# VikParuchuri/surya

Measured on AMD Instinct MI355X. Metric: text-lines/sec recognised (whole node), higher is better.
Workload: dtype bf16; 1 GPU; RecognitionPredictor device loop, 256 ragged 64x{128..512} crops/GPU, batch 256, max_tokens=48, REC-FULL synthetic weights (conditioned recipe, seed 0), tiles resident in HBM; parallelism=1 GPU, weights=conditioned

## Files before the change

### include/surya_amd.h

```cpp
#ifndef SURYA_AMD_H
#define SURYA_AMD_H
#include <stddef.h>
#include <stdint.h>

#ifdef __cplusplus
extern "C" {
#endif

#define SA_OK 0
#define SA_ERR_ARG (-1)
#define SA_ERR_SHAPE (-2)
#define SA_ERR_UNSUPPORTED (-3)
#define SA_ERR_STATE (-4)
#define SA_ERR_NOMEM (-5)

#define SA_DTYPE_F32 0
#define SA_DTYPE_BF16 1

const char* surya_amd_version(void);

typedef struct surya_rec_config {
    int32_t enc_depth, enc_hidden, enc_inter, enc_inter_pad, enc_heads;
    int32_t patch_dim, patch_dim_pad;
    int32_t merge;
    int32_t window_tokens;
    int32_t enc_out_hidden;
    uint32_t fullatt_mask;
    float enc_eps;
    int32_t vocab, dec_hidden, dec_inter, dec_layers, dec_heads, dec_kv_heads, dec_head_dim;
    float dec_eps;
    int32_t bbox_size, embed_multiplier;
    int32_t image_token_id, pad_token_id, eos_token_id;
    int32_t max_slots;
    int32_t max_kv_len;
    int32_t max_patches;
    int32_t max_prefill_tokens;
    int32_t dtype;
} surya_rec_config;

enum {
    SA_RW_PATCH = 0, SA_RW_MERGER_LN, SA_RW_FC1_W, SA_RW_FC1_B, SA_RW_FC2_W, SA_RW_FC2_B, SA_RW_IMG_H, SA_RW_IMG_W,
    SA_RW_DEC_NORM, SA_RW_TOK_EMBED, SA_RW_LM_W, SA_RW_LM_B, SA_RW_BBOX_W, SA_RW_BBOX_B, SA_RW_ENC_INVFREQ,
    SA_RW_DEC_INVFREQ, SA_RW_GLOBALS
};
enum { SA_RE_NORM1 = 0, SA_RE_QKV_W, SA_RE_QKV_B, SA_RE_PROJ_W, SA_RE_PROJ_B, SA_RE_NORM2, SA_RE_GU_W, SA_RE_GU_B,
       SA_RE_DOWN_W, SA_RE_DOWN_B, SA_RE_COUNT };
enum { SA_RD_LN1 = 0, SA_RD_QKV_W, SA_RD_QKV_B, SA_RD_O_W, SA_RD_LN2, SA_RD_GU_W, SA_RD_DOWN_W, SA_RD_COUNT };
#define SA_RW_ENC(l, k) (SA_RW_GLOBALS + (l) * SA_RE_COUNT + (k))
#define SA_RW_DEC(cfg_enc_depth, l, k) (SA_RW_GLOBALS + (cfg_enc_depth) * SA_RE_COUNT + (l) * SA_RD_COUNT + (k))
#define SA_RW_TOTAL(enc_depth, dec_layers) (SA_RW_GLOBALS + (enc_depth) * SA_RE_COUNT + (dec_layers) * SA_RD_COUNT)

typedef struct surya_rec surya_rec;

size_t surya_rec_workspace_bytes(const surya_rec_config* cfg);

int surya_rec_create(const surya_rec_config* cfg, const void* const* weights, int n_weights, surya_rec** out);
int surya_rec_destroy(surya_rec* h);

int surya_rec_plan_encoder(const surya_rec_config* cfg, const int32_t* grid_hw, int n_images, int32_t* src_row,
                           int32_t* pos_hw, int32_t* cu_window, int32_t* n_windows, int32_t* merged_src);

int surya_rec_prefill(surya_rec* h, const float* tiles, const int32_t* grid_hw, int n_images, const int32_t* input_ids,
                      const int32_t* seq_offsets, const int32_t* slot_ids, int n_seqs, void* stream);

int surya_rec_encode_ahead(surya_rec* h, const float* tiles, const int32_t* grid_hw, int n_images, void* stream);

int surya_rec_set_active(surya_rec* h, const int32_t* slots, int n_active, void* stream);

#define SA_MAX_STEPS 16
int surya_rec_decode(surya_rec* h, int n_steps, void* stream);

int surya_rec_read_outputs(surya_rec* h, int n_steps, int32_t* tokens, float* scores, int32_t* bboxes, void* stream);

int surya_rec_decode_async(surya_rec* h, int n_steps, int ring, void* stream);
int surya_rec_wait_outputs(surya_rec* h, int n_steps, int ring, int32_t* tokens, float* scores, int32_t* bboxes);

int surya_rec_preprocess(const uint8_t* pages, const void* lines, int n_lines, uint8_t* mask_arena, float* mid_arena, float* tiles,
                         int patch_size, int merge_size, float pad_value, const float* mean, const float* std, int any_poly,
                         int max_stage1_width, int pixel_stride, void* stream);

int surya_rec_encode_only(surya_rec* h, const float* tiles, const int32_t* grid_hw, int n_images, void* out, void* stream);
int surya_rec_copy_last_logits(surya_rec* h, float* dst, int max_rows, int* rows, void* stream);
int surya_rec_set_next_tokens(surya_rec* h, const int32_t* slots, const int32_t* tokens, int n, void* stream);

enum { SA_MX_QKV_W = 0, SA_MX_QKV_S, SA_MX_O_W, SA_MX_O_S, SA_MX_GU_W, SA_MX_GU_S, SA_MX_DOWN_W, SA_MX_DOWN_S, SA_MX_COUNT };
enum { SA_MX_LM_W = 0, SA_MX_LM_S, SA_MX_GLOBALS };
#define SA_MX_TOTAL(dec_layers) ((dec_layers) * SA_MX_COUNT + SA_MX_GLOBALS)
int surya_rec_set_mx_weights(surya_rec* h, const void* const* table, int n);

int surya_rec_set_kv_fp8(surya_rec* h, int on);

int surya_op_gemm(int dtype, int out_f32, int epi, const void* X, long ldx, const void* W, long ldw, void* C, long ldc,
                  const void* bias, const void* R, long ldr, int M, int N, int K, void* stream);
int surya_op_rmsnorm(int dtype, const void* x, long ldx, const void* w, void* y, long ldy, int rows, int C, float eps,
                     void* stream);
int surya_op_attn(int dtype, int head_dim, const void* q, const void* k, const void* v, void* out, const int32_t* seg_len,
                  const int64_t* q_off, const int64_t* k_off, const int64_t* v_off, const int64_t* o_off, int n_seg, int heads, int group,
                  int causal, float scale, long q_row, long q_head, long k_row, long k_head, long o_row, long o_head, void* stream);
int surya_op_decode_attn(int dtype, int head_dim, const float* qkv_part, int n_slabs, const void* qkv_bias, void* out, void* kcache,
                         void* vcache, const int32_t* active_slots, const int32_t* row_len, const float* rope_cs, int rows, int heads,
                         int kv_heads, int max_kv_len, float scale, void* stream);
int surya_op_kv8_quant_rows(int head_dim, const void* kcache, const void* vcache, const int32_t* tok_slot, const int32_t* tok_pos, int n_tokens,
                            void* k8, void* v8t, float* kscale, float* vscale, int kv_heads, int max_kv_len, void* stream);
int surya_op_decode_attn_kv8(int head_dim, const float* qkv_part, int n_slabs, const void* qkv_bias, void* out, void* k8, void* v8t,
                             float* kscale, float* vscale, const int32_t* active_slots, const int32_t* row_len, const float* rope_cs, int rows,
                             int heads, int kv_heads, int max_kv_len, float scale, void* stream);

int surya_op_mx_quantize(const float* x, int rows, int K, uint8_t* q, uint8_t* scales, void* stream);
int surya_op_gemm_mx(int mode, const uint8_t* X, const uint8_t* SX, const uint8_t* W, const uint8_t* SW, int M, int N, int K,
                     float* C, int* splitk, uint8_t* q_out, uint8_t* sq_out, void* stream);

enum { SA_DET_INPUT = 0,
       SA_DET_CONV,
       SA_DET_DWCONV,
       SA_DET_GROUPED1X1,
       SA_DET_LITEMLA,
       SA_DET_UPCAT,
       SA_DET_CLASSIFY,
       SA_DET_UPSAMPLE_OUT,
       SA_DET_UPSUM_SRC,
       SA_DET_UPSUM_CLASSIFY };
enum { SA_ACT_NONE = 0, SA_ACT_HSWISH = 1, SA_ACT_RELU = 2 };

typedef struct surya_det_op {
    int32_t type;
    int32_t in0, in1, out, res;
    int32_t cin, cout, k, stride, act;
    int32_t hin, win, hout, wout;
    int32_t w_idx, b_idx;
    int32_t p0, p1;
} surya_det_op;

typedef struct surya_det_config {
    int32_t n_ops, max_batch, height, width, num_labels, dtype;
} surya_det_config;

typedef struct surya_det surya_det;

int surya_det_create(const surya_det_config* cfg, const surya_det_op* ops, const void* const* weights, int n_weights,
                     const size_t* buf_elems, int n_bufs, surya_det** out);
int surya_det_destroy(surya_det* h);
int surya_det_forward(surya_det* h, const float* pixel_values, int batch, float* heatmaps, float* lowres, void* stream);
int surya_det_op_count(surya_det* h);
int surya_det_forward_timed(surya_det* h, const float* pixel_values, int batch, float* heatmaps, float* lowres, void* stream, float* op_ms,
                            int n_op_ms);
int surya_det_forward_u8(surya_det* h, const uint8_t* pixels_nhwc, int pixel_stride, const float* mean, const float* std, int batch,
                         float* heatmaps, float* lowres, void* stream);

int surya_resample_lanczos_u8(const uint8_t* src, int src_w, int src_h, int src_pix, uint8_t* dst, int dst_w, int dst_h, int dst_pix,
                              const int32_t* bounds_x, const int32_t* taps_x, int ksize_x, const int32_t* bounds_y,
                              const int32_t* taps_y, int ksize_y, uint8_t* tmp, void* stream);

size_t surya_det_boxes_workspace_bytes(int batch, int height, int width, int max_boxes);
int surya_det_boxes(const float* heat, long page_stride, int batch, int height, int width, float text_threshold, float low_text,
                    int max_boxes, float* boxes, float* conf, int32_t* count, void* workspace, size_t workspace_bytes, void* stream);

typedef struct surya_layout_config {
    int32_t img_h, img_w, patch, embed_dim, n_stages;
    int32_t depths[8], heads[8], kv_heads[8];
    int32_t window;
    float enc_eps;
    int32_t encoder_length;
    int32_t dec_layers, dec_hidden, dec_inter, dec_heads, dec_kv_heads;
    int32_t vocab, label_count, bbox_size;
    float rms_eps, ln_eps;
    int32_t max_batch, max_boxes, dtype;
    int32_t family, box_embed, category_count, merge_count;
} surya_layout_config;
enum { SA_FAMILY_LAYOUT = 0, SA_FAMILY_TABLE = 1 };

enum { SA_LW_PATCH_W = 0, SA_LW_PATCH_B, SA_LW_EMB_LN_W, SA_LW_EMB_LN_B, SA_LW_POS_EMB, SA_LW_DEC_FNORM, SA_LW_DEC_LN_W, SA_LW_DEC_LN_B,
       SA_LW_DEC_LM_W, SA_LW_DEC_BB_W, SA_LW_DEC_BB_B, SA_LW_DEC_INVFREQ, SA_LW_DEC_ZERO_BIAS, SA_LW_EMB_TABLES, SA_LW_GLOBALS = SA_LW_EMB_TABLES + 17 };
enum { SA_LS_SINCOS = 0, SA_LS_MERGE_NORM_W, SA_LS_MERGE_NORM_B, SA_LS_MERGE_RED_W, SA_LS_COUNT };
enum { SA_LB_LN1_W = 0, SA_LB_LN1_B, SA_LB_QKV_W, SA_LB_QKV_B, SA_LB_RELBIAS, SA_LB_PROJ_W, SA_LB_PROJ_B, SA_LB_LN2_W, SA_LB_LN2_B, SA_LB_FC1_W,
       SA_LB_FC1_B, SA_LB_FC2_W, SA_LB_FC2_B, SA_LB_COUNT };
enum { SA_LD_CNORM = 0, SA_LD_CQ_W, SA_LD_CKV_W, SA_LD_CO_W, SA_LD_CO_B, SA_LD_TNORM, SA_LD_QKV_W, SA_LD_TO_W, SA_LD_TO_B, SA_LD_MNORM, SA_LD_GU_W,
       SA_LD_DOWN_W, SA_LD_COUNT };

typedef struct surya_layout surya_layout;
int surya_layout_create(const surya_layout_config* cfg, const void* const* weights, int n_weights, surya_layout** out);
int surya_layout_destroy(surya_layout* h);
int surya_layout_encode(surya_layout* h, const float* pixel_values, int batch, void* stream);
int surya_layout_decode_step(surya_layout* h, const int32_t* boxes, int batch, int position, float* class_logits, float* bbox, void* stream);
int surya_layout_prefill(surya_layout* h, const int32_t* boxes, int batch, int n_tokens, float* class_logits, float* bbox, void* stream);
typedef struct surya_layout_feedback {
    int32_t skew_scaler;
    int32_t relabel_ids[2];
    int32_t head_widths[4];
    const int32_t* page_sizes;
} surya_layout_feedback;
int surya_layout_set_feedback(surya_layout* h, const surya_layout_feedback* fb, int batch, void* stream);
int surya_layout_decode_steps(surya_layout* h, const int32_t* boxes, int batch, int position, int n_steps, int ring, void* stream);
int surya_layout_wait_steps(surya_layout* h, int ring, int batch, int n_steps, float* class_logits, float* bbox, int32_t* fed_tokens);
int surya_layout_select(surya_layout* h, const int32_t* src_index, int n);
int surya_layout_encoder_states(surya_layout* h, void* out, int batch, void* stream);

int surya_prof_enable(int on);
int surya_set_tuning(const char* key, int value);
int surya_prof_read(int max_cfg, int* launches, double* ms, double* flops, double* bytes);
int surya_prof_read2(int max_cfg, int* launches, double* ms, double* flops, double* bytes, double* slab_bytes);
int surya_prof_event_overhead(void* stream, double* ms);

#ifdef __cplusplus
}
#endif
#endif
```

### surya_amd/csrc/common.h

```cpp
#pragma once
#include <hip/hip_runtime.h>
#include <cstdlib>
#include <stdint.h>
#include <stdio.h>

#include "../../include/surya_amd.h"

namespace sa {

typedef unsigned short bf16_t;
typedef __attribute__((ext_vector_type(4))) float f32x4;
typedef __attribute__((ext_vector_type(16))) float f32x16;
typedef __attribute__((ext_vector_type(8))) __bf16 bf16x8;
typedef unsigned int u32x4 __attribute__((ext_vector_type(4)));


#define SA_HIP(expr)                                                                                   \
    do {                                                                                               \
        hipError_t _e = (expr);                                                                        \
        if (_e != hipSuccess) {                                                                        \
            fprintf(stderr, "[surya_amd] %s:%d %s -> %s\n", __FILE__, __LINE__, #expr, hipGetErrorString(_e)); \
            return (int)_e;                                                                            \
        }                                                                                              \
    } while (0)
// ... 62 lines not shown
    v += dpp_mov<0x141>(v);
    v += dpp_mov<0x140>(v);
    return v;
}

__device__ __forceinline__ int mx_block_exp(float absmax) {
    if (!(absmax > 0.f)) return -127;
    int ex;
    const float f = frexpf(absmax, &ex);
    const int e = (f <= 0.875f) ? ex - 9 : ex - 8;
    return max(-127, min(127, e));
}
__device__ __forceinline__ uint32_t mx_pack4(float a, float b, float c, float d) {
    int r = __builtin_amdgcn_cvt_pk_fp8_f32(a, b, 0, false);
    r = __builtin_amdgcn_cvt_pk_fp8_f32(c, d, r, true);
    return (uint32_t)r;
}
template <int CTRL>
__device__ __forceinline__ float dpp_max(float v) { return fmaxf(v, dpp_mov<CTRL>(v)); }
__device__ __forceinline__ float quad_max(float v) { return dpp_max<0x4E>(dpp_max<0xB1>(v)); }
__device__ __forceinline__ float oct_max(float v) { return dpp_max<0x141>(quad_max(v)); }
__device__ __forceinline__ uint32_t mx_quant4_oct(const float (&v)[4], int& e8) {
    const float m = oct_max(fmaxf(fmaxf(fabsf(v[0]), fabsf(v[1])), fmaxf(fabsf(v[2]), fabsf(v[3]))));
    const int e = mx_block_exp(m);
    e8 = e + 127;
    return mx_pack4(ldexpf(v[0], -e), ldexpf(v[1], -e), ldexpf(v[2], -e), ldexpf(v[3], -e));
}

__device__ __forceinline__ float wave_sum(float v) {
#pragma unroll
    for (int o = 32; o > 0; o >>= 1) v += __shfl_xor(v, o, 64);
    return v;
}
__device__ __forceinline__ float wave_max(float v) {
#pragma unroll
    for (int o = 32; o > 0; o >>= 1) v = fmaxf(v, __shfl_xor(v, o, 64));
    return v;
}

__device__ __forceinline__ float silu_f(float x) { return x / (1.0f + __expf(-x)); }
template <typename TI>
__device__ __forceinline__ float silu_epi(float x) {
    if constexpr (sizeof(TI) == 2) return x * __builtin_amdgcn_rcpf(1.0f + __expf(-x));
    else return silu_f(x);
}
__device__ __forceinline__ float gelu_erf_f(float x) { return 0.5f * x * (1.0f + erff(x * 0.70710678118654752440f)); }
template <typename TI>
__device__ __forceinline__ float gelu_epi(float x) {
    if constexpr (sizeof(TI) == 2) {
        const float z = fabsf(x) * 0.70710678118654752440f;
        const float t = __builtin_amdgcn_rcpf(fmaf(0.3275911f, z, 1.0f));
        const float poly = t * fmaf(t, fmaf(t, fmaf(t, fmaf(t, 1.061405429f, -1.453152027f), 1.421413741f), -0.284496736f), 0.254829592f);
        const float erfc_abs = poly * __expf(-z * z);
        return 0.5f * x * (x < 0.f ? erfc_abs : 2.0f - erfc_abs);
    } else {
        return gelu_erf_f(x);
    }
}
__device__ __forceinline__ float gelu_tanh_f(float x) { return 0.5f * x * (1.0f + tanhf(0.7978845608028654f * (x + 0.044715f * x * x * x))); }
__device__ __forceinline__ float sigmoid_f(float x) { return 1.0f / (1.0f + __expf(-x)); }
__device__ __forceinline__ float hardswish_f(float x) {
    float t;
    asm("v_fma_f32 %0, %1, %2, 0.5 clamp" : "=v"(t) : "v"(x), "s"(1.0f / 6.0f));
    return x * t;
}
typedef float f32x2_hs __attribute__((ext_vector_type(2)));
__device__ __forceinline__ f32x2_hs hardswish_pk(f32x2_hs x) {
    f32x2_hs t;
    const f32x2_hs c = {1.0f / 6.0f, 1.0f / 6.0f};
    asm("v_pk_fma_f32 %0, %1, %2, 0.5 op_sel_hi:[1,0,0] clamp" : "=v"(t) : "v"(x), "s"(c));
    return x * t;
}

struct Tuning {
    int graph = 0;
    int split_target = 256;
    int split_min_kt = 4;
    int split_max = 8;
    int bigtile = 3;
    int bigtile_any = 0;
    int big_m_split = -1;
    int big_m_gateup = -1;
    int gateup_ring = 2;
    int conv_persist = 3;
    int dwconv_pipe = 2;
    int conv_lean = 1;
    int bigtile_ratio_pct = 0;
    int bigtile_min_k = 0;
    int glds = 2;
    int dattn = 4;
    int rnorm = 2;
    int ghead = 2;
    int fuse_embed = 1;
    int kvprefetch = 0;
    int lmhead = 1;
    int dattn_db = 0;
    int lay_ln = 1;
    int det_head_blk = 1;
    int det_fuse = 1023;
    int det_up4 = 1;
    int fmb_chunk = 64;
    int persist = 1;
};
inline Tuning& tuning() { static Tuning t; return t; }
inline int& tuning_epoch() { static int e = 0; return e; }

inline void poison_arena(void* p, size_t bytes) {
    static const bool on = [] { const char* e = getenv("SURYA_AMD_POISON"); return e && e[0] == '1'; }();
    if (on) { (void)hipMemset(p, 0xFF, bytes); (void)hipDeviceSynchronize(); }
}

struct AttrOnce {
    size_t granted[64] = {};
    template <typename F> void ensure(F kern, size_t lds) {
        int dev = 0;
        (void)hipGetDevice(&dev);
        size_t& g = granted[dev & 63];
        if (lds > g || g == 0) {
            (void)hipFuncSetAttribute(reinterpret_cast<const void*>(kern), hipFuncAttributeMaxDynamicSharedMemorySize, (int)lds);
            g = lds > g ? lds : g;
            if (g == 0) g = 1;
        }
    }
};

static inline int cdiv(int a, int b) { return (a + b - 1) / b; }
static inline long cdivl(long a, long b) { return (a + b - 1) / b; }

}
```

### surya_amd/csrc/gemm.h

```cpp
#pragma once
#include <algorithm>
#include <cstdlib>
#include <type_traits>

#include "common.h"
#include "fastdiv.h"

namespace sa {

enum GemmEpi { EPI_BIAS = 0, EPI_RESIDUAL = 1, EPI_GELU = 2, EPI_SWIGLU = 3, EPI_HARDSWISH = 4, EPI_RELU = 5, EPI_ARGMAX = 6, EPI_ROPE = 7,
               EPI_GEGLU = 8  };

template <typename TI, typename TO>
struct GemmArgs {
    const TI* X; long ldx;
    const TI* W; long ldw;
    TO* C; long ldc;
    const TI* bias;
    const TO* R; long ldr;
    int M, N, K;
    int splitk = 1;
    float* part = nullptr;
    int swz_m = 0, swz_n = 0;
    int mgroup = 0;
// ... 1178 lines not shown
inline int gemm_cfg_id(int BM, int BN) { return (BM >= 128 && BN >= 128) ? 0 : (BM == 256 ? 1 : 2); }

template <typename TI, typename TO, int BM, int BN, int WM, int WN, int EPI, bool SPLIT = false, int GLDS = 0, bool CONV = false, int WAUX = 0>
static inline int launch_gemm_cfg(const GemmArgs<TI, TO>& a, hipStream_t s) {
    int tiles = SPLIT ? cdiv(cdiv(a.N, BN) * a.splitk, 8) * 8 * cdiv(a.M, BM) : cdiv(a.M, BM) * cdiv(a.N, BN);
    a.bn_used = BN;
    GemmArgs<TI, TO> aa = a;
    if (!SPLIT && BM >= 128 && BN >= 128) {
        const int tm = cdiv(a.M, BM), tn = cdiv(a.N, BN);
        constexpr int GRP = ((BM + BN) * 128 * (GLDS > 2 && GLDS != 8 ? GLDS : 2) > 80 * 1024) ? 32 : 64;
        if (tm * tn >= 8 * GRP) {
            aa.swz_n = cdiv(tn, cdiv(tn, 8));
            aa.swz_m = std::max(1, GRP / aa.swz_n);
            tiles = cdiv(tm * tn, 8 * GRP) * 8 * GRP;
        }
    }
    if (!SPLIT && aa.mgroup) tiles = cdiv(cdiv(a.N, BN), 8) * 8 * cdiv(a.M, BM);
    constexpr size_t out_w = ((EPI == EPI_SWIGLU || EPI == EPI_GEGLU) && !SPLIT) ? BN / 2 : BN;
    constexpr size_t out_bytes = (size_t)BM * out_w * (SPLIT ? sizeof(float) : sizeof(TO));
    constexpr size_t stage_bytes = (size_t)(BM + BN) * 128 * (GLDS > 2 && GLDS != 8 ? GLDS : 2);
    constexpr bool argmax_direct = (EPI == EPI_ARGMAX) && ((size_t)BM * BN * 4 > 160 * 1024);
    constexpr size_t lds = (argmax_direct || stage_bytes > out_bytes) ? stage_bytes : out_bytes;
    auto kern = gemm_nt_kernel<TI, TO, BM, BN, WM, WN, EPI, SPLIT, GLDS, CONV, WAUX>;
    static AttrOnce attr;
    attr.ensure(kern, lds);
    GemmProfiler& pf = gemm_profiler();
    const bool prof = pf.enabled && pf.n < GemmProfiler::POOL;
    if (prof) (void)hipEventRecord(pf.ev[2 * pf.n], s);
    hipLaunchKernelGGL(kern, dim3(tiles), dim3(64 * WM * WN), lds, s, aa);
    if (prof) {
        (void)hipEventRecord(pf.ev[2 * pf.n + 1], s);
        pf.cfg_of[pf.n] = CONV ? 3 : gemm_cfg_id(BM, BN);
        pf.flops_of[pf.n] = CONV ? 2.0 * a.M * a.N * a.cTaps * a.cCin : 2.0 * a.M * a.N * a.K;
        const double outn = (EPI == EPI_SWIGLU || EPI == EPI_GEGLU) ? a.N / 2 : (EPI == EPI_ARGMAX ? 4.0 * cdiv(a.N, BN) : a.N);
        const double xelems = CONV ? (double)a.M / std::max(1, a.cHo * a.cWo) * a.cH * a.cW * a.cCin : (double)a.M * a.K;
        pf.bytes_of[pf.n] = (xelems + (double)a.N * a.K) * sizeof(TI) + (double)a.M * outn * (SPLIT ? sizeof(TI) : sizeof(TO)) +
                            (EPI == EPI_RESIDUAL ? (double)a.M * a.N * sizeof(TO) : 0.0);
        pf.slab_of[pf.n] = SPLIT ? (double)a.splitk * a.M * a.N * 4.0 : 0.0;
        ++pf.n;
    }
    return (int)hipGetLastError();
}

template <typename TI, typename TO, int EPI, int CONV = 0>
static inline int launch_gemm_persist(const GemmArgs<TI, TO>& a, hipStream_t s) {
    constexpr int BM = 256, BN = 256, GRP = 32;
    const int tm = cdiv(a.M, BM), tn = cdiv(a.N, BN);
    GemmArgs<TI, TO> aa = a;
    a.bn_used = BN;
    aa.swz_n = cdiv(tn, cdiv(tn, 8));
    aa.swz_m = std::max(1, GRP / aa.swz_n);
    const int padded = cdiv(tm * tn, 8 * GRP) * 8 * GRP;
    static int n_cu_of[64] = {};
    int dev = 0;
    (void)hipGetDevice(&dev);
    int& n_cu = n_cu_of[dev & 63];
    if (!n_cu) {
        if (hipDeviceGetAttribute(&n_cu, hipDeviceAttributeMultiprocessorCount, dev) != hipSuccess || n_cu <= 0) n_cu = 256;
        n_cu = (n_cu / 8) * 8;
    }
    const int grid = std::min(padded, n_cu);
    constexpr size_t lds = (size_t)2 * (BM + BN) * 128 + 8 * 4096;
    auto kern = gemm_nt_p8p_kernel<TI, TO, EPI, CONV>;
    static AttrOnce attr;
    attr.ensure(kern, lds);
    GemmProfiler& pf = gemm_profiler();
    const bool prof = pf.enabled && pf.n < GemmProfiler::POOL;
    if (prof) (void)hipEventRecord(pf.ev[2 * pf.n], s);
    hipLaunchKernelGGL(kern, dim3(grid), dim3(512), lds, s, aa);
    if (prof) {
        (void)hipEventRecord(pf.ev[2 * pf.n + 1], s);
        pf.cfg_of[pf.n] = CONV ? 3 : gemm_cfg_id(BM, BN);
        pf.flops_of[pf.n] = CONV ? 2.0 * a.M * a.N * a.cTaps * a.cCin : 2.0 * a.M * a.N * a.K;
        const double outn = (EPI == EPI_SWIGLU || EPI == EPI_GEGLU) ? a.N / 2 : a.N;
        const double xelems = CONV ? (double)a.M / std::max(1, a.cHo * a.cWo) * a.cH * a.cW * a.cCin : (double)a.M * a.K;
        pf.bytes_of[pf.n] = (xelems + (double)a.N * a.K) * sizeof(TI) + (double)a.M * outn * sizeof(TO) +
                            (EPI == EPI_RESIDUAL ? (double)a.M * a.N * sizeof(TO) : 0.0);
        pf.slab_of[pf.n] = 0.0;
        ++pf.n;
    }
    return (int)hipGetLastError();
}

template <typename TI, typename TO, int EPI>
static inline int launch_gemm(const GemmArgs<TI, TO>& a, hipStream_t s) {
    if (a.M <= 0 || a.N <= 0) return SA_OK;
    {
        const int n_out = (EPI == EPI_SWIGLU || EPI == EPI_GEGLU) ? a.N / 2 : a.N;
        if (a.K % Ty<TI>::KE != 0 || a.N % 4 != 0 || n_out % (16 / (int)sizeof(TO)) != 0 || a.ldc % (16 / (int)sizeof(TO)) != 0)
            return SA_ERR_SHAPE;
    }
    if (a.M <= 256) {
        if constexpr (EPI == EPI_ARGMAX) {
            if (a.N >= 64 * 512 && tuning().lmhead && (a.K / Ty<TI>::KE) % 2 == 0 && a.N % 4 == 0) {
                if constexpr (sizeof(TI) == 2)
                    if (tuning().lmhead == 2) return launch_gemm_cfg<TI, TO, 256, 320, 4, 2, EPI, false, 2, false, 2>(a, s);
                return launch_gemm_cfg<TI, TO, 256, 320, 4, 2, EPI, false, 2>(a, s);
            }
            if (a.N >= 64 * 512) return launch_gemm_cfg<TI, TO, 128, 128, 2, 2, EPI, false, 2>(a, s);
            return launch_gemm_cfg<TI, TO, 64, 64, 2, 2, EPI, false, 2>(a, s);
        }
        if (a.M > 128) {
            if (a.N >= 64 * 512) return launch_gemm_cfg<TI, TO, 128, 128, 2, 2, EPI, false, 2>(a, s);
            if constexpr (EPI == EPI_SWIGLU && sizeof(TI) == 2) {
                if (tuning().gateup_ring == 3) return launch_gemm_cfg<TI, TO, 64, 64, 2, 2, EPI, false, 3>(a, s);
                if (tuning().gateup_ring == 4) return launch_gemm_cfg<TI, TO, 64, 64, 2, 2, EPI, false, 4>(a, s);
            }
            return launch_gemm_cfg<TI, TO, 64, 64, 2, 2, EPI, false, 2>(a, s);
        }
        if (a.M > 64) {
            if (a.N >= 64 * 128) return launch_gemm_cfg<TI, TO, 128, 64, 4, 1, EPI>(a, s);
            return launch_gemm_cfg<TI, TO, 128, 32, 4, 1, EPI>(a, s);
        }
        if (a.N >= 64 * 128) return launch_gemm_cfg<TI, TO, 64, 64, 2, 2, EPI>(a, s);
        return launch_gemm_cfg<TI, TO, 64, 32, 2, 1, EPI>(a, s);
    }
    if constexpr (EPI == EPI_ARGMAX) {
        if (a.N >= 64 * 512 && tuning().lmhead && (a.K / Ty<TI>::KE) % 2 == 0 && a.N % 4 == 0) {
            GemmArgs<TI, TO> g = a;
            g.mgroup = 1;
            int rc;
            if constexpr (sizeof(TI) == 2) {
                if (tuning().lmhead == 2) { rc = launch_gemm_cfg<TI, TO, 256, 320, 4, 2, EPI, false, 2, false, 2>(g, s); a.bn_used = g.bn_used; return rc; }
            }
            rc = launch_gemm_cfg<TI, TO, 256, 320, 4, 2, EPI, false, 2>(g, s);
            a.bn_used = g.bn_used;
            return rc;
        }
    }
    if constexpr (EPI == EPI_SWIGLU && sizeof(TI) == 2 && sizeof(TO) == 2) {
        const int mode = tuning().big_m_gateup;
        const int rb = cdiv(a.M, 256), t256 = rb * cdiv(a.N, 256);
        const int pick = mode >= 0 ? mode : ((rb >= 4 && t256 >= 160 && t256 < 256) ? 2 : 0);
        if (pick && (a.K / Ty<TI>::KE) % 2 == 0 && a.K / Ty<TI>::KE >= 4 && a.N % 8 == 0) {
            if (pick == 1) return launch_gemm_persist<TI, TO, EPI>(a, s);
            return launch_gemm_cfg<TI, TO, 256, 256, 4, 2, EPI, false, 8>(a, s);
        }
    }
    if (a.N <= 64 && a.M >= 128 * 256) return launch_gemm_cfg<TI, TO, 128, 64, 4, 1, EPI>(a, s);
    const long big = (long)cdiv(a.M, 128) * cdiv(a.N, 128);
    const int glds = tuning().glds;
    if constexpr (sizeof(TO) == 2) {
        const int bigtile = tuning().bigtile;
        const long t256 = (long)cdiv(a.M, 256) * cdiv(a.N, 256);
        const double ratio256 = tuning().bigtile_ratio_pct > 0 ? tuning().bigtile_ratio_pct / 100.0
                                                                : ((bigtile == 3 && sizeof(TI) == 2) ? 1.4 : 1.17);
        const double cost256 = (double)cdivl(t256, 256) * 256 * 4 / ratio256, cost128 = (double)cdivl(big, 512) * 512;
        if (bigtile && a.K >= tuning().bigtile_min_k && ((t256 >= 256 && cost256 <= cost128) || tuning().bigtile_any)) {
            if constexpr (EPI != EPI_ARGMAX) {
                const int nk = a.K / Ty<TI>::KE;
                if constexpr (sizeof(TI) == 2)
                    if (tuning().persist && nk >= 4 && nk % 2 == 0 && a.N % 8 == 0) return launch_gemm_persist<TI, TO, EPI>(a, s);
            }
            if constexpr (sizeof(TI) == 2 && EPI != EPI_ARGMAX) {
                if (bigtile == 2) return launch_gemm_cfg<TI, TO, 256, 256, 2, 2, EPI, false, 2>(a, s);
                if (bigtile == 3 && (a.K / Ty<TI>::KE) % 2 == 0) return launch_gemm_cfg<TI, TO, 256, 256, 4, 2, EPI, false, 8>(a, s);
            }
            return launch_gemm_cfg<TI, TO, 256, 256, 4, 2, EPI, false, 2>(a, s);
        }
    }
    if (big >= 256) {
        if (glds == 2) return launch_gemm_cfg<TI, TO, 128, 128, 2, 2, EPI, false, 2>(a, s);
        if (glds == 3) return launch_gemm_cfg<TI, TO, 128, 128, 2, 2, EPI, false, 3>(a, s);
        return launch_gemm_cfg<TI, TO, 128, 128, 2, 2, EPI>(a, s);
    }
    return launch_gemm_cfg<TI, TO, 64, 64, 2, 2, EPI>(a, s);
}

static inline int pick_splitk(int tiles_n, int nk) {
    const Tuning& t = tuning();
    const int tiles = tiles_n * 4;
    int s = (t.split_target + tiles / 2) / tiles;
    s = std::min(s, nk / std::max(1, t.split_min_kt));
    return std::max(1, std::min(s, std::min(t.split_max, 8)));
}

template <typename TI>
static inline int launch_gemm_splitk(GemmArgs<TI, TI>& a, hipStream_t s) {
    if (a.M <= 0 || a.N <= 0) return SA_OK;
    if (a.K % Ty<TI>::KE != 0 || a.N % 4 != 0 || !a.part) return SA_ERR_SHAPE;
    const int nk = a.K / Ty<TI>::KE;
    a.splitk = pick_splitk(cdiv(a.N, 64), nk);
    if constexpr (sizeof(TI) == 2) {
        const int mode = tuning().big_m_split;
        const int w128 = cdiv(a.M, 128) * cdiv(a.N, 128) * a.splitk, w12864 = cdiv(a.M, 128) * cdiv(a.N, 64) * a.splitk;
        const int pick = a.M <= 256 ? 0 : (mode >= 0 ? mode : (w128 >= 136 ? 2 : (w12864 <= 256 ? 3 : 0)));
        if (pick == 2) return launch_gemm_cfg<TI, TI, 128, 128, 2, 2, EPI_BIAS, true, 4>(a, s);
        if (pick == 3) return launch_gemm_cfg<TI, TI, 128, 64, 4, 1, EPI_BIAS, true, 4>(a, s);
    }
    return launch_gemm_cfg<TI, TI, 64, 64, 2, 2, EPI_BIAS, true, 4>(a, s);
}

}
```

### surya_amd/csrc/rec_model.hip

```cpp
#include <algorithm>
#include <cstdlib>
#include <cstring>
#include <map>
#include <memory>
#include <set>
#include <vector>

#include "../../include/surya_amd.h"
#include "gemm.h"
#include "gemm_mx.h"
#include "kernels.h"
#include "decode_attn.h"
#include "decode_attn_kv8.h"
#include "attn_mfma.h"
#include "rec_prep.h"

namespace sa {

struct Stager {
    char* host = nullptr;
    char* dev = nullptr;
    size_t cap = 0, off = 0;
    hipEvent_t ev = nullptr;
    bool pending = false;
// ... 1229 lines not shown
        else if (d == 64 && G <= 8) SA_OPD_FLASH(64, 8)
        else if (d == 32 && G <= 8) SA_OPD_FLASH(32, 8)
        else return SA_ERR_UNSUPPORTED;
    } else if (dtype == SA_DTYPE_F32) {
        if (d == 128 && G <= 5) SA_OPD_MFMA(128, 5)
        else if (d == 128 && G <= 8) SA_OPD_MFMA(128, 8)
        else if (d == 64 && G <= 8) SA_OPD_MFMA(64, 8)
        else if (d == 32 && G <= 8) SA_OPD_MFMA(32, 8)
        else return SA_ERR_UNSUPPORTED;
    } else {
        return SA_ERR_UNSUPPORTED;
    }
#undef SA_OPD_FLASH
#undef SA_OPD_FLASH3
#undef SA_OPD_FLASH4
#undef SA_OPD_MFMA
#undef SA_OPD
    return (int)hipGetLastError();
}

int surya_op_kv8_quant_rows(int head_dim, const void* kcache, const void* vcache, const int32_t* tok_slot, const int32_t* tok_pos, int n_tokens,
                            void* k8, void* v8t, float* kscale, float* vscale, int kv_heads, int max_kv_len, void* stream) {
    if (!kcache || !vcache || !tok_slot || !tok_pos || !k8 || !v8t || !kscale || !vscale || n_tokens <= 0 || kv_heads <= 0) return SA_ERR_ARG;
    hipStream_t s = (hipStream_t)stream;
    const int T8 = (max_kv_len + 255) & ~255;
    dim3 qg(cdiv(n_tokens * kv_heads, 4));
#define SA_Q8(DD)                                                                                                                  \
    hipLaunchKernelGGL(kv8_quant_rows_kernel<DD>, qg, dim3(256), 0, s, (const bf16_t*)kcache, (const bf16_t*)vcache, tok_slot, tok_pos, \
                       n_tokens, (uint8_t*)k8, (uint8_t*)v8t, kscale, vscale, kv_heads, max_kv_len, T8)
    if (head_dim == 128) SA_Q8(128);
    else if (head_dim == 64) SA_Q8(64);
    else if (head_dim == 32) SA_Q8(32);
    else return SA_ERR_UNSUPPORTED;
#undef SA_Q8
    return (int)hipGetLastError();
}

int surya_op_decode_attn_kv8(int head_dim, const float* qkv_part, int n_slabs, const void* qkv_bias, void* out, void* k8, void* v8t,
                             float* kscale, float* vscale, const int32_t* active_slots, const int32_t* row_len, const float* rope_cs, int rows,
                             int heads, int kv_heads, int max_kv_len, float scale, void* stream) {
    if (!qkv_part || !qkv_bias || !out || !k8 || !v8t || !kscale || !vscale || !active_slots || !row_len || !rope_cs) return SA_ERR_ARG;
    if (rows <= 0 || n_slabs < 1 || n_slabs > 8 || kv_heads <= 0 || heads % kv_heads) return SA_ERR_ARG;
    hipStream_t s = (hipStream_t)stream;
    const int G = heads / kv_heads, d = head_dim, T8 = (max_kv_len + 255) & ~255;
    dim3 grid(rows, kv_heads), block(256);
    const float2* cs = reinterpret_cast<const float2*>(rope_cs);
#define SA_OPD8(DD, GG)                                                                                                          \
    {                                                                                                                           \
        auto kern = decode_attn_kv8_kernel<DD, GG>;                                                                             \
        static AttrOnce attr;                                                                                                   \
        attr.ensure(kern, decode_attn_kv8_lds<DD, GG>());                                                                       \
        hipLaunchKernelGGL(kern, grid, dim3(KV8_THREADS), (decode_attn_kv8_lds<DD, GG>()), s, qkv_part, n_slabs, (const bf16_t*)qkv_bias, \
                           (bf16_t*)out, (uint8_t*)k8, (uint8_t*)v8t, kscale, vscale, active_slots, row_len, cs, heads, kv_heads, \
                           max_kv_len, T8, scale, (uint8_t*)nullptr, (uint8_t*)nullptr, 0);                                     \
    }
    if (d == 128 && G <= 5) SA_OPD8(128, 5)
    else if (d == 128 && G <= 8) SA_OPD8(128, 8)
    else if (d == 64 && G <= 8) SA_OPD8(64, 8)
    else if (d == 32 && G <= 8) SA_OPD8(32, 8)
    else return SA_ERR_UNSUPPORTED;
#undef SA_OPD8
    return (int)hipGetLastError();
}

__global__ __launch_bounds__(256) void mx_quantize_rows_kernel(const float* __restrict__ x, int K, uint8_t* __restrict__ q,
                                                               uint8_t* __restrict__ sc) {
    const long row = blockIdx.x, rows = gridDim.x;
    for (int c = threadIdx.x * 4; c < K; c += 1024) {
        float v[4];
        load4(x + row * K + c, v);
        int e8;
        const uint32_t pk = mx_quant4_oct(v, e8);
        *reinterpret_cast<uint32_t*>(q + row * K + c) = pk;
        if ((threadIdx.x & 7) == 0) sc[((long)(c >> 7) * rows + row) * 4 + ((c >> 5) & 3)] = (uint8_t)e8;
    }
}

int surya_op_mx_quantize(const float* x, int rows, int K, uint8_t* q, uint8_t* scales, void* stream) {
    if (!x || !q || !scales || rows <= 0 || K <= 0 || K % 128) return SA_ERR_ARG;
    hipLaunchKernelGGL(mx_quantize_rows_kernel, dim3(rows), dim3(256), 0, (hipStream_t)stream, x, K, q, scales);
    return (int)hipGetLastError();
}

int surya_op_gemm_mx(int mode, const uint8_t* X, const uint8_t* SX, const uint8_t* W, const uint8_t* SW, int M, int N, int K,
                     float* C, int* splitk, uint8_t* q_out, uint8_t* sq_out, void* stream) {
    if (!X || !SX || !W || !SW) return SA_ERR_ARG;
    MxArgs a{X, (long)K, SX, W, (long)K, SW, M, N, K, (long)M, (long)N};
    hipStream_t s = (hipStream_t)stream;
    if (mode == 0) {
        if (!C) return SA_ERR_ARG;
        a.C = C; a.ldc = N;
        return launch_gemm_mx<MX_EPI_F32>(a, s);
    }
    if (mode == 1) {
        if (!C || !splitk) return SA_ERR_ARG;
        a.part = C;
        int rc = launch_gemm_mx_splitk(a, s);
        *splitk = a.splitk;
        return rc;
    }
    if (mode == 2) {
        if (!q_out || !sq_out) return SA_ERR_ARG;
        a.Q = q_out; a.ldq = N / 2; a.SQ = sq_out; a.sq_rows = M;
        return launch_gemm_mx<MX_EPI_SWIGLU>(a, s);
    }
    return SA_ERR_ARG;
}

int surya_rec_preprocess(const uint8_t* pages, const void* lines, int n_lines, uint8_t* mask_arena, float* mid_arena, float* tiles,
                         int patch_size, int merge_size, float pad_value, const float* mean, const float* std, int any_poly,
                         int max_stage1_width, int pixel_stride, void* stream) {
    if (!pages || !lines || !tiles || !mean || !std || n_lines < 0 || patch_size <= 0 || merge_size <= 0) return SA_ERR_ARG;
    if (pixel_stride != 3 && pixel_stride != 4) return SA_ERR_ARG;
    sa::prep::PrepArgs p;
    p.pages = pages; p.lines = reinterpret_cast<const sa::prep::LineDesc*>(lines); p.n_lines = n_lines;
    p.mask = mask_arena; p.mid = mid_arena; p.tiles = tiles; p.ps = patch_size; p.merge = merge_size; p.pad = pad_value;
    for (int i = 0; i < 3; ++i) { p.mean[i] = mean[i]; p.std[i] = std[i]; }
    p.max_mid_w = max_stage1_width;
    p.pix = pixel_stride;
    return sa::prep::prep_run(p, any_poly, max_stage1_width > 0, (hipStream_t)stream);
}

int surya_set_tuning(const char* key, int value) {
    if (!key) return SA_ERR_ARG;
    Tuning& t = tuning();
    struct { const char* k; int* v; } tab[] = {
        {"graph", &t.graph}, {"split_target", &t.split_target}, {"split_min_kt", &t.split_min_kt}, {"split_max", &t.split_max},
        {"bigtile", &t.bigtile}, {"bigtile_any", &t.bigtile_any}, {"conv_lean", &t.conv_lean}, {"conv_persist", &t.conv_persist}, {"dwconv_pipe", &t.dwconv_pipe}, {"bigtile_ratio_pct", &t.bigtile_ratio_pct}, {"gateup_ring", &t.gateup_ring}, {"big_m_split", &t.big_m_split}, {"big_m_gateup", &t.big_m_gateup}, {"glds", &t.glds}, {"bigtile_min_k", &t.bigtile_min_k}, {"dattn", &t.dattn}, {"rnorm", &t.rnorm},
        {"ghead", &t.ghead}, {"fuse_embed", &t.fuse_embed}, {"persist", &t.persist}, {"lmhead", &t.lmhead}, {"kvprefetch", &t.kvprefetch},
        {"dattn_db", &t.dattn_db}, {"lay_ln", &t.lay_ln}, {"det_head_blk", &t.det_head_blk}, {"det_fuse", &t.det_fuse}, {"det_up4", &t.det_up4}, {"fmb_chunk", &t.fmb_chunk}};
    for (auto& e : tab)
        if (!strcmp(e.k, key)) {
            if (*e.v != value) ++tuning_epoch();
            *e.v = value;
            return SA_OK;
        }
    return SA_ERR_ARG;
}

int surya_prof_enable(int on) {
    GemmProfiler& pf = gemm_profiler();
    if (on) pf.start(); else pf.enabled = false;
    return SA_OK;
}

__global__ void prof_null_kernel() {}

int surya_prof_event_overhead(void* stream, double* ms) {
    if (!ms) return SA_ERR_ARG;
    hipStream_t s = (hipStream_t)stream;
    constexpr int N = 201;
    hipEvent_t ev[2 * N];
    for (auto& e : ev) SA_HIP(hipEventCreate(&e));
    for (int i = 0; i < 32; ++i) hipLaunchKernelGGL(prof_null_kernel, dim3(1), dim3(64), 0, s);
    for (int i = 0; i < N; ++i) {
        SA_HIP(hipEventRecord(ev[2 * i], s));
        hipLaunchKernelGGL(prof_null_kernel, dim3(1), dim3(64), 0, s);
        SA_HIP(hipEventRecord(ev[2 * i + 1], s));
    }
    SA_HIP(hipStreamSynchronize(s));
    std::vector<float> t(N);
    for (int i = 0; i < N; ++i) SA_HIP(hipEventElapsedTime(&t[i], ev[2 * i], ev[2 * i + 1]));
    for (auto& e : ev) (void)hipEventDestroy(e);
    std::sort(t.begin(), t.end());
    *ms = t[N / 2];
    return SA_OK;
}

int surya_prof_read2(int max_cfg, int* launches, double* ms, double* flops, double* bytes, double* slab_bytes) {
    GemmProfiler& pf = gemm_profiler();
    if (!launches || !ms || !flops || !bytes || max_cfg < GemmProfiler::NCFG) return SA_ERR_ARG;
    SA_HIP(hipDeviceSynchronize());
    for (int c = 0; c < GemmProfiler::NCFG; ++c) { launches[c] = 0; ms[c] = flops[c] = bytes[c] = 0.0; if (slab_bytes) slab_bytes[c] = 0.0; }
    for (int i = 0; i < pf.n; ++i) {
        float t = 0.f;
        SA_HIP(hipEventElapsedTime(&t, pf.ev[2 * i], pf.ev[2 * i + 1]));
        const int c = pf.cfg_of[i];
        launches[c]++; ms[c] += t; flops[c] += pf.flops_of[i]; bytes[c] += pf.bytes_of[i];
        if (slab_bytes) slab_bytes[c] += pf.slab_of[i];
    }
    pf.n = 0;
    return SA_OK;
}

int surya_prof_read(int max_cfg, int* launches, double* ms, double* flops, double* bytes) {
    return surya_prof_read2(max_cfg, launches, ms, flops, bytes, nullptr);
}

int surya_op_rmsnorm(int dtype, const void* x, long ldx, const void* w, void* y, long ldy, int rows, int C, float eps,
                     void* stream) {
    if (!x || !w || !y || rows <= 0) return SA_ERR_ARG;
    hipStream_t s = (hipStream_t)stream;
    if (dtype == SA_DTYPE_F32)
        hipLaunchKernelGGL(rmsnorm_kernel<float>, dim3(cdiv(rows, 4)), dim3(256), 0, s, (const float*)x, ldx, (const float*)w,
                           (float*)y, ldy, (const int*)nullptr, rows, C, eps);
    else if (dtype == SA_DTYPE_BF16)
        hipLaunchKernelGGL(rmsnorm_kernel<bf16_t>, dim3(cdiv(rows, 4)), dim3(256), 0, s, (const bf16_t*)x, ldx, (const bf16_t*)w,
                           (bf16_t*)y, ldy, (const int*)nullptr, rows, C, eps);
    else
        return SA_ERR_UNSUPPORTED;
    return (int)hipGetLastError();
}

}
```

Measured before the change: 3160 lines/s.

## Add warp-specialized producer/consumer ring GEMM for decode gate-up projections

Adds a GEMM kernel in which dedicated loader waves stream X/W tiles into a multi-slot LDS ring using global_load_lds. Compute waves consume the slots via LDS full/free flag words and issue MFMAs, so loads and math overlap without block-wide barriers. With default tuning (dring=1, M in 129..256) it is used for the SwiGLU gate-up GEMM. The split-K variant is off by default because dring_min_kt=0. The spin-wait has a limit and an error word to catch deadlocks, which adds risk and an extra status API.

```diff
diff --git a/include/surya_amd.h b/include/surya_amd.h
--- a/include/surya_amd.h
+++ b/include/surya_amd.h
@@ -106,6 +106,7 @@
                              float* kscale, float* vscale, const int32_t* active_slots, const int32_t* row_len, const float* rope_cs, int rows,
                              int heads, int kv_heads, int max_kv_len, float scale, void* stream);
 
+int surya_op_gemm_splitk_bf16(const void* X, long ldx, const void* W, long ldw, float* part, int M, int N, int K, int* splitk, void* stream);
 int surya_op_mx_quantize(const float* x, int rows, int K, uint8_t* q, uint8_t* scales, void* stream);
 int surya_op_gemm_mx(int mode, const uint8_t* X, const uint8_t* SX, const uint8_t* W, const uint8_t* SW, int M, int N, int K,
                      float* C, int* splitk, uint8_t* q_out, uint8_t* sq_out, void* stream);
@@ -197,6 +198,7 @@
 
 int surya_prof_enable(int on);
 int surya_set_tuning(const char* key, int value);
+int surya_gemm_ring_status(int reset);
 int surya_prof_read(int max_cfg, int* launches, double* ms, double* flops, double* bytes);
 int surya_prof_read2(int max_cfg, int* launches, double* ms, double* flops, double* bytes, double* slab_bytes);
 int surya_prof_event_overhead(void* stream, double* ms);
diff --git a/surya_amd/csrc/common.h b/surya_amd/csrc/common.h
--- a/surya_amd/csrc/common.h
+++ b/surya_amd/csrc/common.h
@@ -168,6 +168,8 @@
     int big_m_split = -1;
     int big_m_gateup = -1;
     int gateup_ring = 2;
+    int dring = 1;
+    int dring_min_kt = 0;
     int conv_persist = 3;
     int dwconv_pipe = 2;
     int conv_lean = 1;
diff --git a/surya_amd/csrc/gemm.h b/surya_amd/csrc/gemm.h
--- a/surya_amd/csrc/gemm.h
+++ b/surya_amd/csrc/gemm.h
@@ -1284,6 +1284,10 @@
     return (int)hipGetLastError();
 }
 
+}
+#include "gemm_ring.h"
+namespace sa {
+
 template <typename TI, typename TO, int EPI>
 static inline int launch_gemm(const GemmArgs<TI, TO>& a, hipStream_t s) {
     if (a.M <= 0 || a.N <= 0) return SA_OK;
@@ -1304,6 +1308,10 @@
         }
         if (a.M > 128) {
             if (a.N >= 64 * 512) return launch_gemm_cfg<TI, TO, 128, 128, 2, 2, EPI, false, 2>(a, s);
+            if constexpr (EPI == EPI_SWIGLU && sizeof(TI) == 2 && sizeof(TO) == 2) {
+                const int rc = launch_gateup_ring(a, s);
+                if (rc >= 0) return rc;
+            }
             if constexpr (EPI == EPI_SWIGLU && sizeof(TI) == 2) {
                 if (tuning().gateup_ring == 3) return launch_gemm_cfg<TI, TO, 64, 64, 2, 2, EPI, false, 3>(a, s);
                 if (tuning().gateup_ring == 4) return launch_gemm_cfg<TI, TO, 64, 64, 2, 2, EPI, false, 4>(a, s);
@@ -1390,6 +1398,10 @@
         if (pick == 2) return launch_gemm_cfg<TI, TI, 128, 128, 2, 2, EPI_BIAS, true, 4>(a, s);
         if (pick == 3) return launch_gemm_cfg<TI, TI, 128, 64, 4, 1, EPI_BIAS, true, 4>(a, s);
     }
+    if constexpr (sizeof(TI) == 2) {
+        const int rc = launch_splitk_ring(a, s);
+        if (rc >= 0) return rc;
+    }
     return launch_gemm_cfg<TI, TI, 64, 64, 2, 2, EPI_BIAS, true, 4>(a, s);
 }
 
diff --git a/surya_amd/csrc/gemm_ring.h b/surya_amd/csrc/gemm_ring.h
--- /dev/null
+++ b/surya_amd/csrc/gemm_ring.h
@@ -0,0 +1,244 @@
+#pragma once
+
+namespace sa {
+
+static __device__ unsigned ring_error_word;
+
+template <int EPI, int BM, int BN, int CWM, int CWN, int NL, int SLOTS, bool SPLIT, int WAUX>
+__global__ __launch_bounds__(64 * (CWM * CWN + NL)) void gemm_ring_kernel(GemmArgs<bf16_t, bf16_t> p) {
+    using TI = bf16_t;
+    using TO = bf16_t;
+    constexpr int NC = CWM * CWN;
+    constexpr int WTM = BM / CWM, WTN = BN / CWN, FM = WTM / 32, FN = WTN / 32;
+    constexpr int XG = BM / 8, G = (BM + BN) / 8, GPW = G / NL;
+    constexpr int SLOT = (BM + BN) * 128;
+    constexpr int FLAGS = SLOTS * SLOT;
+    constexpr unsigned SPIN_LIMIT = 1u << 20;
+    static_assert(FM >= 1 && FN >= 1 && WTM % 32 == 0 && WTN % 32 == 0 && G % NL == 0, "ring tile");
+    static_assert(SLOTS >= 5 && 2 * GPW <= 63, "ring depth / vmcnt range");
+    static_assert(!(EPI == EPI_SWIGLU) || !SPLIT, "gated epilogue on full-K tiles only");
+    extern __shared__ __attribute__((aligned(16))) unsigned char smem[];
+    typedef const __attribute__((address_space(1))) void* gptr_t;
+    typedef __attribute__((address_space(3))) void* lptr_t;
+
+    const int tid = threadIdx.x, lane = tid & 63;
+    const int wave = __builtin_amdgcn_readfirstlane(tid >> 6);
+    const int tiles_n = (p.N + BN - 1) / BN, tiles_m = (p.M + BM - 1) / BM, S = SPLIT ? p.splitk : 1;
+    const int x8 = (int)blockIdx.x & 7, j8 = (int)blockIdx.x >> 3;
+    const int pair = (j8 / tiles_m) * 8 + x8;
+    if (pair >= tiles_n * S) return;
+    const int tile_m = j8 % tiles_m, tile_n = pair / S, ks = pair % S;
+    const int m0 = tile_m * BM, n0 = tile_n * BN;
+    const int nk_all = p.K / Ty<TI>::KE;
+    const int kt_begin = SPLIT ? (int)((long)ks * nk_all / p.splitk) : 0;
+    const int kt_end = SPLIT ? (int)((long)(ks + 1) * nk_all / p.splitk) : nk_all;
+    const int nk = kt_end - kt_begin;
+
+    const unsigned lds0 = (unsigned)(size_t)(lptr_t)smem;
+    const unsigned full_w = lds0 + FLAGS, free_w = full_w + SLOTS * NL * 4;
+    if (tid < SLOTS * (NL + NC)) reinterpret_cast<unsigned*>(smem + FLAGS)[tid] = 0u;
+    __syncthreads();
+
+    bool broken = false;
+    auto wait_words = [&](unsigned base, int n, unsigned target) {
+        const unsigned addr = base + (unsigned)(lane % n) * 4u;
+        for (unsigned spin = 0; !broken; ++spin) {
+            unsigned v;
+            asm volatile("ds_read_b32 %0, %1\n\ts_waitcnt lgkmcnt(0)" : "=v"(v) : "v"(addr) : "memory");
+            if (__builtin_amdgcn_ballot_w64(v < target) == 0) break;
+            if (spin >= SPIN_LIMIT) {
+                broken = true;
+                if (lane == 0) atomicOr(&ring_error_word, 1u);
+                break;
+            }
+            __builtin_amdgcn_s_sleep(1);
+        }
+    };
+    auto post_word = [&](unsigned addr, unsigned v) { asm volatile("ds_write_b32 %0, %1" ::"v"(addr), "v"(v) : "memory"); };
+
+    f32x16 acc[FN][FM];
+    if (wave >= NC) {
+        const int lw = wave - NC;
+        const unsigned char* src[GPW];
+#pragma unroll
+        for (int i = 0; i < GPW; ++i) {
+            const int g = lw * GPW + i;
+            const int lr = (g < XG ? g : g - XG) * 8 + (lane >> 3), c = (lane & 7) ^ ((lr >> 1) & 7);
+            const unsigned char* base = g < XG ? reinterpret_cast<const unsigned char*>(p.X + (long)min(m0 + lr, p.M - 1) * p.ldx)
+                                               : reinterpret_cast<const unsigned char*>(p.W + (long)min(n0 + lr, p.N - 1) * p.ldw);
+            src[i] = base + c * 16 + (long)kt_begin * 128;
+        }
+        const unsigned my_full = full_w + lw * 4;
+        int slot = 0, lap = 0;
+        for (int kt = 0; kt < nk; ++kt) {
+            if (kt >= SLOTS) wait_words(free_w + slot * NC * 4, NC, (unsigned)lap);
+            const long koff = (long)kt * 128;
+#pragma unroll
+            for (int i = 0; i < GPW; ++i) {
+                const int g = lw * GPW + i;
+                unsigned char* dst = smem + slot * SLOT + g * 1024;
+                if (WAUX == 0 || g < XG) __builtin_amdgcn_global_load_lds((gptr_t)(src[i] + koff), (lptr_t)dst, 16, 0, 0);
+                else __builtin_amdgcn_global_load_lds((gptr_t)(src[i] + koff), (lptr_t)dst, 16, 0, WAUX);
+            }
+            if (kt >= 2) {
+                asm volatile("s_waitcnt vmcnt(%0)" ::"n"(2 * GPW) : "memory");
+                const int ps = slot >= 2 ? slot - 2 : slot + SLOTS - 2;
+                post_word(my_full + ps * NL * 4, (unsigned)((kt - 2) / SLOTS + 1));
+            }
+            if (++slot == SLOTS) { slot = 0; ++lap; }
+        }
+        if (nk >= 2) {
+            asm volatile("s_waitcnt vmcnt(%0)" ::"n"(GPW) : "memory");
+            const int kt = nk - 2;
+            post_word(my_full + (kt % SLOTS) * NL * 4, (unsigned)(kt / SLOTS + 1));
+        }
+        if (nk >= 1) {
+            asm volatile("s_waitcnt vmcnt(0)" ::: "memory");
+            const int kt = nk - 1;
+            post_word(my_full + (kt % SLOTS) * NL * 4, (unsigned)(kt / SLOTS + 1));
+        }
+    } else {
+        const int cm = wave / CWN, cn = wave % CWN;
+        const int frow = lane & 31, fch = lane >> 5;
+#pragma unroll
+        for (int j = 0; j < FN; ++j)
+#pragma unroll
+            for (int i = 0; i < FM; ++i)
+#pragma unroll
+                for (int r = 0; r < 16; ++r) acc[j][i][r] = 0.f;
+        int xo[FM], wo[FN];
+        int xs[FM], ws[FN];
+#pragma unroll
+        for (int i = 0; i < FM; ++i) {
+            const int row = cm * WTM + i * 32 + frow;
+            xo[i] = row * 128; xs[i] = (row >> 1) & 7;
+        }
+#pragma unroll
+        for (int j = 0; j < FN; ++j) {
+            const int row = cn * WTN + j * 32 + frow;
+            wo[j] = BM * 128 + row * 128; ws[j] = (row >> 1) & 7;
+        }
+        const unsigned my_free = free_w + wave * 4;
+        int slot = 0, lap = 0;
+        for (int kt = 0; kt < nk; ++kt) {
+            wait_words(full_w + slot * NL * 4, NL, (unsigned)(lap + 1));
+            asm volatile("" ::: "memory");
+            const unsigned char* cur = smem + slot * SLOT;
+            u32x4 xf[4][FM], wf[4][FN];
+#pragma unroll
+            for (int kk = 0; kk < 4; ++kk) {
+#pragma unroll
+                for (int i = 0; i < FM; ++i) xf[kk][i] = *reinterpret_cast<const u32x4*>(cur + xo[i] + (((kk * 2 + fch) ^ xs[i]) << 4));
+#pragma unroll
+                for (int j = 0; j < FN; ++j) wf[kk][j] = *reinterpret_cast<const u32x4*>(cur + wo[j] + (((kk * 2 + fch) ^ ws[j]) << 4));
+            }
+            asm volatile("s_waitcnt lgkmcnt(0)" ::: "memory");
+            post_word(my_free + slot * NC * 4, (unsigned)(lap + 1));
+#pragma unroll
+            for (int kk = 0; kk < 4; ++kk)
+#pragma unroll
+                for (int j = 0; j < FN; ++j)
+#pragma unroll
+                    for (int i = 0; i < FM; ++i) Mfma<TI>::run(acc[j][i], wf[kk][j], xf[kk][i]);
+            if (++slot == SLOTS) { slot = 0; ++lap; }
+        }
+    }
+    __syncthreads();
+
+    constexpr bool GLU = (EPI == EPI_SWIGLU);
+    constexpr int OW = GLU ? BN / 2 : BN;
+    constexpr int ES = SPLIT ? 4 : 2;
+    constexpr int ROWB = OW * ES, PITCH = ROWB + 16, CPR = ROWB / 16, EPC = 16 / ES;
+    static_assert(ROWB % 16 == 0 && BM * PITCH <= SLOTS * SLOT, "output staging");
+    if (wave < NC) {
+        const int cm = wave / CWN, cn = wave % CWN;
+#pragma unroll
+        for (int i = 0; i < FM; ++i) {
+            const int row = cm * WTM + i * 32 + (lane & 31);
+#pragma unroll
+            for (int j = 0; j < FN; ++j)
+#pragma unroll
+                for (int g = 0; g < 4; ++g) {
+                    const int ncol = cn * WTN + j * 32 + g * 8 + (lane >> 5) * 4;
+                    const float v0 = acc[j][i][4 * g], v1 = acc[j][i][4 * g + 1], v2 = acc[j][i][4 * g + 2], v3 = acc[j][i][4 * g + 3];
+                    if constexpr (GLU) {
+                        store2(reinterpret_cast<TO*>(smem + row * PITCH + (ncol >> 1) * ES), silu_epi<TI>(v0) * v1, silu_epi<TI>(v2) * v3);
+                    } else if constexpr (SPLIT) {
+                        store4(reinterpret_cast<float*>(smem + row * PITCH + ncol * ES), v0, v1, v2, v3);
+                    } else {
+                        store4(reinterpret_cast<TO*>(smem + row * PITCH + ncol * ES), v0, v1, v2, v3);
+                    }
+                }
+        }
+    }
+    __syncthreads();
+    constexpr int NT = 64 * (NC + NL);
+    const int n_out = GLU ? p.N / 2 : p.N, n0_out = GLU ? n0 / 2 : n0;
+    for (int id = tid; id < BM * CPR; id += NT) {
+        const int row = id / CPR, c = id % CPR;
+        const int m = m0 + row, n = n0_out + c * EPC;
+        if (m >= p.M || n >= n_out) continue;
+        const u32x4 raw = *reinterpret_cast<const u32x4*>(smem + row * PITCH + c * 16);
+        if constexpr (SPLIT) *reinterpret_cast<u32x4*>(p.part + ((long)ks * p.M + m) * p.N + n) = raw;
+        else *reinterpret_cast<u32x4*>(p.C + (long)m * p.ldc + n) = raw;
+    }
+}
+
+template <int EPI, int BM, int BN, int CWM, int CWN, int NL, int SLOTS, bool SPLIT, int WAUX>
+static inline int launch_gemm_ring(const GemmArgs<bf16_t, bf16_t>& a, hipStream_t s) {
+    const int S = SPLIT ? a.splitk : 1;
+    const int grid = cdiv(cdiv(a.N, BN) * S, 8) * 8 * cdiv(a.M, BM);
+    constexpr int NT = 64 * (CWM * CWN + NL);
+    constexpr size_t lds = (size_t)SLOTS * (BM + BN) * 128 + (size_t)SLOTS * (NL + CWM * CWN) * 4;
+    static_assert(lds <= 160 * 1024 && SLOTS * (NL + CWM * CWN) <= NT, "ring LDS / flag clear");
+    a.bn_used = BN;
+    auto kern = gemm_ring_kernel<EPI, BM, BN, CWM, CWN, NL, SLOTS, SPLIT, WAUX>;
+    static AttrOnce attr;
+    attr.ensure(kern, lds);
+    GemmProfiler& pf = gemm_profiler();
+    const bool prof = pf.enabled && pf.n < GemmProfiler::POOL;
+    if (prof) (void)hipEventRecord(pf.ev[2 * pf.n], s);
+    hipLaunchKernelGGL(kern, dim3(grid), dim3(NT), lds, s, a);
+    if (prof) {
+        (void)hipEventRecord(pf.ev[2 * pf.n + 1], s);
+        pf.cfg_of[pf.n] = gemm_cfg_id(BM, BN);
+        pf.flops_of[pf.n] = 2.0 * a.M * a.N * a.K;
+        const double outn = EPI == EPI_SWIGLU ? a.N / 2 : a.N;
+        pf.bytes_of[pf.n] = ((double)a.M * a.K + (double)a.N * a.K) * 2.0 + (double)a.M * outn * 2.0;
+        pf.slab_of[pf.n] = SPLIT ? (double)a.splitk * a.M * a.N * 4.0 : 0.0;
+        ++pf.n;
+    }
+    return (int)hipGetLastError();
+}
+
+static inline int ring_mode(int M) {
+    const int d = tuning().dring;
+    if (!(d & 3) || M <= 0 || M > 256) return 0;
+    if (M <= 128 && !(d & 4)) return 0;
+    return d & 3;
+}
+static inline int launch_gateup_ring(const GemmArgs<bf16_t, bf16_t>& a, hipStream_t s) {
+    const int mode = ring_mode(a.M);
+    if (!mode || a.bias || a.N % 8 != 0) return -1;
+    if (mode == 2) return launch_gemm_ring<EPI_SWIGLU, 64, 160, 1, 5, 4, 5, false, 2>(a, s);
+    return launch_gemm_ring<EPI_SWIGLU, 64, 160, 1, 5, 4, 5, false, 0>(a, s);
+}
+static inline int launch_splitk_ring(const GemmArgs<bf16_t, bf16_t>& a, hipStream_t s) {
+    const int mode = ring_mode(a.M);
+    const int min_kt = tuning().dring_min_kt;
+    if (!mode || min_kt <= 0 || (a.K / Ty<bf16_t>::KE) / a.splitk < min_kt) return -1;
+    if (mode == 2) return launch_gemm_ring<EPI_BIAS, 64, 64, 2, 2, 4, 8, true, 2>(a, s);
+    return launch_gemm_ring<EPI_BIAS, 64, 64, 2, 2, 4, 8, true, 0>(a, s);
+}
+
+static inline int ring_error(bool reset) {
+    unsigned v = 0;
+    if (hipMemcpyFromSymbol(&v, HIP_SYMBOL(ring_error_word), sizeof(v)) != hipSuccess) return SA_ERR_STATE;
+    if (reset && v) {
+        const unsigned z = 0;
+        (void)hipMemcpyToSymbol(HIP_SYMBOL(ring_error_word), &z, sizeof(z));
+    }
+    return v ? SA_ERR_STATE : SA_OK;
+}
+
+}
diff --git a/surya_amd/csrc/rec_model.hip b/surya_amd/csrc/rec_model.hip
--- a/surya_amd/csrc/rec_model.hip
+++ b/surya_amd/csrc/rec_model.hip
@@ -1335,6 +1335,14 @@
     return (int)hipGetLastError();
 }
 
+int surya_op_gemm_splitk_bf16(const void* X, long ldx, const void* W, long ldw, float* part, int M, int N, int K, int* splitk, void* stream) {
+    if (!X || !W || !part || !splitk) return SA_ERR_ARG;
+    GemmArgs<bf16_t, bf16_t> a{reinterpret_cast<const bf16_t*>(X), ldx, reinterpret_cast<const bf16_t*>(W), ldw, nullptr, 0, nullptr, nullptr, 0, M, N, K, 1, part};
+    const int rc = launch_gemm_splitk<bf16_t>(a, (hipStream_t)stream);
+    *splitk = a.splitk;
+    return rc;
+}
+
 int surya_op_gemm_mx(int mode, const uint8_t* X, const uint8_t* SX, const uint8_t* W, const uint8_t* SW, int M, int N, int K,
                      float* C, int* splitk, uint8_t* q_out, uint8_t* sq_out, void* stream) {
     if (!X || !SX || !W || !SW) return SA_ERR_ARG;
@@ -1379,7 +1387,7 @@
     Tuning& t = tuning();
     struct { const char* k; int* v; } tab[] = {
         {"graph", &t.graph}, {"split_target", &t.split_target}, {"split_min_kt", &t.split_min_kt}, {"split_max", &t.split_max},
-        {"bigtile", &t.bigtile}, {"bigtile_any", &t.bigtile_any}, {"conv_lean", &t.conv_lean}, {"conv_persist", &t.conv_persist}, {"dwconv_pipe", &t.dwconv_pipe}, {"bigtile_ratio_pct", &t.bigtile_ratio_pct}, {"gateup_ring", &t.gateup_ring}, {"big_m_split", &t.big_m_split}, {"big_m_gateup", &t.big_m_gateup}, {"glds", &t.glds}, {"bigtile_min_k", &t.bigtile_min_k}, {"dattn", &t.dattn}, {"rnorm", &t.rnorm},
+        {"bigtile", &t.bigtile}, {"bigtile_any", &t.bigtile_any}, {"conv_lean", &t.conv_lean}, {"conv_persist", &t.conv_persist}, {"dwconv_pipe", &t.dwconv_pipe}, {"bigtile_ratio_pct", &t.bigtile_ratio_pct}, {"gateup_ring", &t.gateup_ring}, {"dring", &t.dring}, {"dring_min_kt", &t.dring_min_kt}, {"big_m_split", &t.big_m_split}, {"big_m_gateup", &t.big_m_gateup}, {"glds", &t.glds}, {"bigtile_min_k", &t.bigtile_min_k}, {"dattn", &t.dattn}, {"rnorm", &t.rnorm},
         {"ghead", &t.ghead}, {"fuse_embed", &t.fuse_embed}, {"persist", &t.persist}, {"lmhead", &t.lmhead}, {"kvprefetch", &t.kvprefetch},
         {"dattn_db", &t.dattn_db}, {"lay_ln", &t.lay_ln}, {"det_head_blk", &t.det_head_blk}, {"det_fuse", &t.det_fuse}, {"det_up4", &t.det_up4}, {"fmb_chunk", &t.fmb_chunk}};
     for (auto& e : tab)
@@ -1390,6 +1398,8 @@
         }
     return SA_ERR_ARG;
 }
+
+int surya_gemm_ring_status(int reset) { return sa::ring_error(reset != 0); }
 
 int surya_prof_enable(int on) {
     GemmProfiler& pf = gemm_profiler();
```

New measurement: 3218 lines/s, median of 6. 1.8% higher.
